# rusty-fast-solvers/rusty-compression

Measured on AMD Instinct MI355X. Metric: GB/s + compressions/sec, 8192x8192 f64 rank-128 rSVD+ID, higher is better.
Workload: dtype f64

## Files before the change

### rusty_compression_amd/csrc/kernels_gemm.hip

```cpp
#include "rc_common.hpp"
#include "rc_gemm.hpp"

#include <cstdlib>
#include <type_traits>

namespace rc {


constexpr int pitch16(int n) { return n + ((16 - n % 32) + 32) % 32; }
constexpr int pitch4(int n) { return n + ((4 - n % 8) + 8) % 8; }

template <typename T, int LAY, int R, int BK, int NT, int VEC, int MODE = 0>
struct TileStager {
    static constexpr int P = LAY == 0 ? (MODE == 0 ? BK + 2 : BK + 8) : (MODE == 0 ? pitch16(R) : pitch4(R));
    static constexpr int ELEMS = LAY == 0 ? R * P : BK * P;
    static constexpr int NVEC = R * BK / VEC;
    static constexpr int PER_T = (NVEC + NT - 1) / NT;
    typedef typename Acc<T>::vec2 vec2;

    const T *ptr[PER_T];
    T val[PER_T][VEC];

    static __device__ inline void coords(int idx, int &r, int &k) {
        if (LAY == 0) { k = (idx % (BK / VEC)) * VEC; r = idx / (BK / VEC); }
// ... 339 lines not shown
    }
}

template <typename T>
__global__ __launch_bounds__(256) void k_splitk_reduce_t(GemmArgs<T> g) {
    __shared__ T tile[32][33];
    const int tx = threadIdx.x & 31, ty = threadIdx.x >> 5;
    const int64_t n0 = (int64_t)blockIdx.x * 32, m0 = (int64_t)blockIdx.y * 32;
#pragma unroll
    for (int r = 0; r < 4; ++r) {
        const int64_t gm = m0 + ty + 8 * r, gn = n0 + tx;
        T s = 0;
        if (gm < g.M && gn < g.N) s = slab_sum(g.partial + gm * g.N + gn, g.M * g.N, g.splits);
        tile[ty + 8 * r][tx] = s;
    }
    __syncthreads();
#pragma unroll
    for (int r = 0; r < 4; ++r) {
        const int64_t gm = m0 + tx, gn = n0 + ty + 8 * r;
        if (gm < g.M && gn < g.N) {
            const T s = tile[tx][ty + 8 * r];
            T *cp = g.c + gm * g.scm + gn * g.scn;
            *cp = g.beta == (T)0 ? g.alpha * s : g.alpha * s + g.beta * (*cp);
        }
    }
}

static int wide_target(const rc_context *c, int many, int lone) {
    static const int target_slots = env_int("RC_GEMM_SLOTS_TARGET", 128);
    const int n = c->lanes_in_flight();
    return n >= 8 ? many : n >= 2 ? target_slots : lone;
}

template <typename T, int BK, class Pipe>
static void launch_split(rc_context *c, GemmArgs<T> g, int target, int min_ksteps, void (*kern)(GemmArgs<T>), int nt, size_t lds,
                         bool (&attr_set)[64], const char *name, Pipe &&pipe) {
    const int64_t tiles = (int64_t)g.tiles_m * g.tiles_n;
    int splits = 1;
    const int64_t ksteps = cdiv(g.K, BK);
    const int min_ks = min_ksteps > 0 ? min_ksteps : (tiles >= 32 ? 16 : 4);
    while (tiles * splits < target && splits < 128 && ksteps / (splits * 2) >= min_ks) splits *= 2;
    g.kchunk = cdiv(cdiv(g.K, splits), BK) * BK;
    splits = (int)cdiv(g.K, g.kchunk);
    if (splits < 1) splits = 1;
    g.splits = splits;
    ArenaMark mark(c);
    if (splits > 1) g.partial = c->alloc<T>((size_t)splits * g.M * g.N);
    if (lds > 48 * 1024 && !attr_set[c->device & 63]) {
        RC_HIP(hipFuncSetAttribute(reinterpret_cast<const void *>(kern), hipFuncAttributeMaxDynamicSharedMemorySize, (int)lds));
        attr_set[c->device & 63] = true;
    }
    c->last_gemm_kernel = name;
    if (!pipe(g)) {
        ProfScope ps(c, "kernel:k_gemm_mfma<%s> M=%lld N=%lld K=%lld", sizeof(T) == 8 ? "f64" : "f32", (long long)g.M, (long long)g.N, (long long)g.K);
        hipLaunchKernelGGL(kern, dim3((unsigned)tiles, (unsigned)splits), dim3(nt), lds, c->stream, g);
    }
    if (splits > 1) {
        ProfScope ps(c, "kernel:k_splitk_reduce M=%lld N=%lld splits=%d", (long long)g.M, (long long)g.N, splits);
        if (g.scm < g.scn && g.N >= 32) {
            hipLaunchKernelGGL(k_splitk_reduce_t<T>, dim3((unsigned)cdiv(g.N, 32), (unsigned)cdiv(g.M, 32)), dim3(256), 0, c->stream, g);
        } else {
            int grid = (int)std::min<int64_t>(cdiv(g.M * g.N, 256), 4096);
            hipLaunchKernelGGL(k_splitk_reduce<T>, dim3(grid), dim3(256), 0, c->stream, g);
        }
    }
}

template <typename T, int ALAY, int BLAY, int BM, int BN, int BK, int WM, int WN, int VEC, int NBUF = 2>
static void launch_cfg(rc_context *c, GemmArgs<T> g, int target_wgs = 0, int min_ksteps = 0) {
    constexpr int NT = WM * WN * 64;
    typedef TileStager<T, ALAY, BM, BK, NT, VEC> StA;
    typedef TileStager<T, BLAY == 1 ? 0 : 1, BN, BK, NT, VEC> StB;
    constexpr size_t lds = NBUF * (size_t)(StA::ELEMS + StB::ELEMS) * sizeof(T);
    static_assert(lds <= 160 * 1024, "tile does not fit LDS");
    g.tiles_m = (int)cdiv(g.M, BM);
    g.tiles_n = (int)cdiv(g.N, BN);
    const int64_t tiles = (int64_t)g.tiles_m * g.tiles_n;
    static const int target_big = env_int("RC_GEMM_TARGET_WGS", 256), target_small = env_int("RC_GEMM_SMALL_TARGET", 32);
    const int target = target_wgs > 0 ? target_wgs : tiles >= 8 ? (tiles >= 32 ? wide_target(c, 1, target_big) : target_big) : target_small;
    static bool attr_set[64] = {};
    char nm[128];
    snprintf(nm, sizeof(nm), "k_gemm_mfma<%s,%d,%d,%d,%d,%d,%d,%d,%d,%d>", sizeof(T) == 8 ? "double" : "float", ALAY, BLAY, BM, BN, BK, WM, WN, VEC, NBUF);
    launch_split<T, BK>(c, g, target, min_ksteps, k_gemm_mfma<T, ALAY, BLAY, BM, BN, BK, WM, WN, VEC, NBUF>, NT, lds, attr_set, nm,
                        [](const GemmArgs<T> &) { return false; });
}

template <int ALAY, int BLAY, int BM, int BN, int BK, int WM, int WN, int VEC, int ORIENT, int GLDS = 0>
static void launch_f64q(rc_context *c, GemmArgs<double> g, int target_wgs = 0, int min_ksteps = 0) {
    typedef double T;
    constexpr int NT = WM * WN * 64;
    typedef TileStager<T, ALAY, BM, BK, NT, VEC> StA;
    typedef TileStager<T, BLAY == 1 ? 0 : 1, BN, BK, NT, VEC> StB;
    constexpr size_t lds = 2 * (size_t)(StA::ELEMS + StB::ELEMS) * sizeof(T);
    static_assert(lds <= 160 * 1024, "tile does not fit LDS");
    g.tiles_m = (int)cdiv(g.M, BM);
    g.tiles_n = (int)cdiv(g.N, BN);
    const int64_t tiles = (int64_t)g.tiles_m * g.tiles_n;
    static const int target_big = env_int("RC_GEMM_TARGET_WGS", 256), target_small = env_int("RC_GEMM_SMALL_TARGET", 32);
    static const int target_lanes = env_int("RC_GEMM_LANES_TARGET", 1);
    const int lone = target_wgs > 0 ? target_wgs : target_big;
    const int target = tiles >= 8 ? (tiles >= 32 ? wide_target(c, target_lanes, lone) : lone) : target_small;
    static bool attr_set[64] = {};
    char nm[128];
    snprintf(nm, sizeof(nm), "k_gemm_f64q<%d,%d,%d,%d,%d,%d,%d,%d,%d,%d>", ALAY, BLAY, BM, BN, BK, WM, WN, VEC, ORIENT, GLDS);
    launch_split<T, BK>(c, g, target, min_ksteps, k_gemm_f64q<ALAY, BLAY, BM, BN, BK, WM, WN, VEC, ORIENT, GLDS>, NT, lds, attr_set, nm,
                        [&](const GemmArgs<T> &gs) { return gemm_f64p_launch(c, gs, ALAY, BLAY, BM, BN, BK, WM, WN, ORIENT, VEC == 2); });
}

template <int ALAY, int BLAY, int VEC>
static void launch_shape_f64q(rc_context *c, const GemmArgs<double> &g) {
    if (g.M <= 144 && g.N <= 144 && g.M > 80 && g.N > 80) launch_f64q<ALAY, BLAY, 144, 144, 16, 3, 3, VEC, 0>(c, g);
    else if (g.N <= 80) launch_f64q<ALAY, BLAY, 256, 80, 16, 8, 1, VEC, 0>(c, g);
    else if (g.N <= 128) launch_f64q<ALAY, BLAY, 256, 128, 16, 8, 1, VEC, 0>(c, g);
    else if (g.N <= 144) launch_f64q<ALAY, BLAY, 256, 144, 16, 8, 1, VEC, 0>(c, g);
    else if (g.M <= 32 && g.K >= 512) {
        launch_f64q<ALAY, BLAY, 32, 256, 16, 1, 8, VEC, 1>(c, g, 512, 4);
    }
    else if (g.M <= 80) launch_f64q<ALAY, BLAY, 80, 256, 16, 1, 8, VEC, 1>(c, g);
    else if (g.M <= 136 && g.K <= 160 && g.N >= 2048) {
        if (g.M <= 128) launch_f64q<ALAY, BLAY, 128, 128, 16, 1, 8, VEC, 1>(c, g);
        else launch_f64q<ALAY, BLAY, 136, 128, 16, 2, 4, VEC, 0>(c, g);
    }
    else if (g.M <= 128) {
        if constexpr (BLAY == 0 && VEC == 2) {
            const bool direct = g.N % 256 == 0 && g.K % 16 == 0 && g.sbn == 1 && g.sbk % 2 == 0 && reinterpret_cast<uintptr_t>(g.b) % 16 == 0;
            if constexpr (ALAY == 1) {
                const bool direct_a = g.M == 128 && g.sam == 1 && g.sak % 2 == 0 && reinterpret_cast<uintptr_t>(g.a) % 16 == 0;
                if (direct && direct_a) { launch_f64q<ALAY, BLAY, 128, 256, 16, 1, 8, VEC, 1, 2>(c, g); return; }
            }
            if (direct) { launch_f64q<ALAY, BLAY, 128, 256, 16, 1, 8, VEC, 1, 1>(c, g); return; }
        }
        launch_f64q<ALAY, BLAY, 128, 256, 16, 1, 8, VEC, 1>(c, g);
    }
    else if (g.M <= 136) launch_f64q<ALAY, BLAY, 136, 256, 16, 2, 4, VEC, 0>(c, g);
    else if (g.M <= 144) launch_f64q<ALAY, BLAY, 144, 256, 16, 1, 8, VEC, 1>(c, g);
    else launch_f64q<ALAY, BLAY, 128, 128, 16, 2, 2, VEC, 0>(c, g);
}

template <typename T, int ALAY, int BLAY, int VEC>
static void launch_shape(rc_context *c, const GemmArgs<T> &g) {
    if constexpr (std::is_same_v<T, double>) {
        launch_shape_f64q<ALAY, BLAY, VEC>(c, g);
    } else {
        constexpr bool panel = ALAY == 0 && BLAY == 1 && VEC == 2;
        if (g.M <= 144 && g.N <= 144 && g.M > 80 && g.N > 80) launch_cfg<T, ALAY, BLAY, 144, 144, 16, 3, 3, VEC>(c, g);
        else if (g.N <= 80) launch_cfg<T, ALAY, BLAY, 128, 80, 16, 4, 1, VEC>(c, g);
        else if (g.N <= 144) launch_cfg<T, ALAY, BLAY, 256, 144, 16, 8, 1, VEC>(c, g);
        else if (panel && g.M <= 32 && g.K >= 512) {
            if constexpr (panel) launch_cfg<T, ALAY, BLAY, 32, 128, 16, 1, 4, VEC>(c, g, 512, 4);
        } else if (g.M <= 80) launch_cfg<T, ALAY, BLAY, 80, 128, 16, 1, 4, VEC>(c, g);
        else if (g.M <= 144) launch_cfg<T, ALAY, BLAY, 144, 256, 16, 1, 8, VEC>(c, g);
        else launch_cfg<T, ALAY, BLAY, 128, 128, 16, 2, 2, VEC>(c, g);
    }
}

template <typename T, int ALAY, int BLAY>
static void launch_vec(rc_context *c, const GemmArgs<T> &g) {
    auto ok = [](const T *p, int64_t s_contig, int64_t s_other) {
        return s_contig == 1 && (s_other % 2) == 0 && (reinterpret_cast<uintptr_t>(p) % (2 * sizeof(T))) == 0;
    };
    const bool va = ALAY == 0 ? ok(g.a, g.sak, g.sam) : ok(g.a, g.sam, g.sak);
    const bool vb = BLAY == 0 ? ok(g.b, g.sbn, g.sbk) : ok(g.b, g.sbk, g.sbn);
    if (va && vb) launch_shape<T, ALAY, BLAY, 2>(c, g);
    else launch_shape<T, ALAY, BLAY, 1>(c, g);
}

template <typename T>
__global__ __launch_bounds__(256) void k_scale_c(Mat<T> cm, T beta) {
    const int64_t total = cm.rows * cm.cols;
    for (int64_t e = blockIdx.x * (int64_t)256 + threadIdx.x; e < total; e += (int64_t)gridDim.x * 256) {
        const int64_t j = e / cm.rows, i = e - j * cm.rows;
        cm.at(i, j) = beta * cm.at(i, j);
    }
}

template <typename T>
void gemm(rc_context *c, T alpha, Mat<T> a, Mat<T> b, T beta, Mat<T> cm) {
    RC_REQUIRE(a.cols == b.rows && a.rows == cm.rows && b.cols == cm.cols, RC_INVALID_ARGUMENT,
               "gemm: shapes (%lld x %lld) * (%lld x %lld) -> (%lld x %lld)", (long long)a.rows, (long long)a.cols,
               (long long)b.rows, (long long)b.cols, (long long)cm.rows, (long long)cm.cols);
    if (cm.empty()) return;
    ArenaMark mark(c);
    if (a.cols == 0) {
        if (beta == (T)0) fill_zero(c, cm);
        else if (beta != (T)1) hipLaunchKernelGGL(k_scale_c<T>, dim3((unsigned)std::min<int64_t>(cdiv(cm.rows * cm.cols, 256), 8192)), dim3(256), 0, c->stream, cm, beta);
        return;
    }
    if (a.rs != 1 && a.cs != 1) {
        T *p = c->alloc<T>((size_t)a.rows * a.cols);
        Mat<T> pa = rowmajor(p, a.rows, a.cols, a.cols);
        copy_mat(c, a, pa);
        a = pa;
    }
    if (b.rs != 1 && b.cs != 1) {
        T *p = c->alloc<T>((size_t)b.rows * b.cols);
        Mat<T> pb = rowmajor(p, b.rows, b.cols, b.cols);
        copy_mat(c, b, pb);
        b = pb;
    }
    if (sizeof(T) == 8 && b.cols <= 144 && a.rows > 144) {
        const Mat<T> a2 = b.t(), b2 = a.t();
        a = a2;
        b = b2;
        cm = cm.t();
    }
    GemmArgs<T> g;
    g.a = a.p; g.b = b.p; g.c = cm.p;
    g.M = a.rows; g.N = b.cols; g.K = a.cols;
    g.sam = a.rs; g.sak = a.cs; g.sbk = b.rs; g.sbn = b.cs; g.scm = cm.rs; g.scn = cm.cs;
    g.alpha = alpha; g.beta = beta;
    g.kchunk = g.K; g.splits = 1; g.partial = nullptr; g.tiles_m = g.tiles_n = 0;
    const bool a_kc = (a.cs == 1);
    const bool b_nc = (b.cs == 1);
    if (a_kc) {
        if (b_nc) launch_vec<T, 0, 0>(c, g); else launch_vec<T, 0, 1>(c, g);
    } else {
        if (b_nc) launch_vec<T, 1, 0>(c, g); else launch_vec<T, 1, 1>(c, g);
    }
}

template void gemm<double>(rc_context *, double, Mat<double>, Mat<double>, double, Mat<double>);
template void gemm<float>(rc_context *, float, Mat<float>, Mat<float>, float, Mat<float>);

}
```

### rusty_compression_amd/csrc/kernels_gemm_pipe.hip

```cpp
#include "rc_gemm.hpp"

#include <type_traits>
#include <utility>

namespace rc {

typedef double pdouble2_t __attribute__((ext_vector_type(2)));
typedef unsigned int pint4_t __attribute__((ext_vector_type(4)));

constexpr int pp_pitch16(int n) { return n + ((16 - n % 32) + 32) % 32; }

template <int LAY, int R, int BK, int NT>
struct PipeStage {
    static constexpr int P = LAY == 0 ? BK + 2 : pp_pitch16(R);
    static constexpr int ELEMS = LAY == 0 ? R * P : BK * P;
    static constexpr int NVEC = R * BK / 2;
    static constexpr int PER_T = (NVEC + NT - 1) / NT;
    static_assert(PER_T * NT <= 2 * NVEC && R % 2 == 0 && BK % 2 == 0, "staging shape");

    uint32_t goff[PER_T];
    pint4_t val[PER_T];

    static __device__ inline void coords(int idx, int &r, int &k) {
        if (idx >= NVEC) idx -= NVEC;
// ... 389 lines not shown
                    g.partial[((int64_t)split * g.M + gm) * g.N + gn] = v;
                } else {
                    double *cp = g.c + gm * g.scm + gn * g.scn;
                    *cp = g.beta == 0.0 ? g.alpha * v : g.alpha * v + g.beta * (*cp);
                }
            }
        }
}

template <int BLAY, int ORIENT, int BM, int BN, int WM, int WN, bool MASKTAIL>
static bool launch_r(rc_context *c, const GemmArgs<double> &g) {
    constexpr int NT = WM * WN * 64;
    constexpr size_t lds = 3 * (size_t)(DirectRows<BM, 16, NT, MASKTAIL>::ELEMS + (BLAY == 0 ? DirectRows<BN, 16, NT>::ELEMS : DirectK<BN, 16, NT>::ELEMS)) * sizeof(double);
    static_assert(lds <= 160 * 1024, "ring does not fit LDS");
    if (g.sam != 1) return false;
    if (BLAY == 0 ? g.sbn != 1 : (g.sbk != 1 || g.N % BN != 0)) return false;
    const int64_t a_span = ((int64_t)256 * g.sam + g.kchunk * g.sak + 2) * 8;
    const int64_t b_span = ((int64_t)BN * g.sbn + g.kchunk * g.sbk + 2) * 8;
    if (a_span >= (1ll << 31) || b_span >= (1ll << 31) || g.sak < 0 || g.sbn < 0 || g.sbk < 0) return false;
    auto kern = k_gemm_f64r<BLAY, ORIENT, BM, BN, WM, WN, MASKTAIL>;
    static bool attr_set[64] = {};
    if (!attr_set[c->device & 63]) {
        RC_HIP(hipFuncSetAttribute(reinterpret_cast<const void *>(kern), hipFuncAttributeMaxDynamicSharedMemorySize, (int)lds));
        attr_set[c->device & 63] = true;
    }
    char nm[128];
    snprintf(nm, sizeof(nm), "k_gemm_f64r<%d,%d,%d,%d,%d,%d,%s,0>", BLAY, ORIENT, BM, BN, WM, WN, MASKTAIL ? "true" : "false");
    c->last_gemm_kernel = nm;
    ProfScope ps(c, "kernel:k_gemm_mfma<f64> M=%lld N=%lld K=%lld", (long long)g.M, (long long)g.N, (long long)g.K);
    hipLaunchKernelGGL(kern, dim3((unsigned)(g.tiles_m * g.tiles_n), (unsigned)g.splits), dim3(NT), lds, c->stream, g);
    return true;
}

template <int ALAY, int BLAY, int BM, int BN, int BK, int WM, int WN, int ORIENT>
static bool launch_p(rc_context *c, const GemmArgs<double> &g) {
    constexpr int NT = WM * WN * 64;
    typedef PipeStage<ALAY, BM, BK, NT> SA;
    typedef PipeStage<BLAY == 1 ? 0 : 1, BN, BK, NT> SB;
    constexpr size_t lds = 2 * (size_t)(SA::ELEMS + SB::ELEMS) * sizeof(double);
    static_assert(lds <= 160 * 1024, "tile does not fit LDS");
    const int64_t a_span = ((int64_t)BM * g.sam + g.kchunk * g.sak + 2) * 8;
    const int64_t b_span = ((int64_t)BN * g.sbn + g.kchunk * g.sbk + 2) * 8;
    if (a_span >= (1ll << 31) || b_span >= (1ll << 31) || g.sam < 0 || g.sak < 0 || g.sbn < 0 || g.sbk < 0) return false;
    auto kern = k_gemm_f64p<ALAY, BLAY, BM, BN, BK, WM, WN, ORIENT>;
    static bool attr_set[64] = {};
    if (lds > 48 * 1024 && !attr_set[c->device & 63]) {
        RC_HIP(hipFuncSetAttribute(reinterpret_cast<const void *>(kern), hipFuncAttributeMaxDynamicSharedMemorySize, (int)lds));
        attr_set[c->device & 63] = true;
    }
    char nm[128];
    snprintf(nm, sizeof(nm), "k_gemm_f64p<%d,%d,%d,%d,%d,%d,%d,%d>", ALAY, BLAY, BM, BN, BK, WM, WN, ORIENT);
    c->last_gemm_kernel = nm;
    ProfScope ps(c, "kernel:k_gemm_mfma<f64> M=%lld N=%lld K=%lld", (long long)g.M, (long long)g.N, (long long)g.K);
    hipLaunchKernelGGL(kern, dim3((unsigned)(g.tiles_m * g.tiles_n), (unsigned)g.splits), dim3(NT), lds, c->stream, g);
    return true;
}

bool gemm_f64p_launch(rc_context *c, const GemmArgs<double> &g, int alay, int blay, int bm, int bn, int bk, int wm, int wn, int orient, bool vec2) {
    if (!vec2 || bk != 16) return false;
    if (g.K % bk != 0 || g.kchunk % bk != 0 || g.K < bk) return false;
    if (alay == 1 && blay == 1 && bm == 136 && bn == 256 && wm == 2 && wn == 4 && orient == 0 && launch_r<1, 0, 136, 256, 2, 4, true>(c, g)) return true;
    if (alay == 1 && blay == 0 && bm == 128 && bn == 256 && wm == 1 && wn == 8 && orient == 1 && launch_r<0, 1, 128, 256, 1, 8, false>(c, g)) return true;
#define RC_PIPE_CASE(AL, BL, BM_, BN_, WM_, WN_, OR_)                                                              \
    if (alay == AL && blay == BL && bm == BM_ && bn == BN_ && wm == WM_ && wn == WN_ && orient == OR_)             \
        return launch_p<AL, BL, BM_, BN_, 16, WM_, WN_, OR_>(c, g);
    RC_PIPE_CASE(0, 1, 144, 144, 3, 3, 0)
    RC_PIPE_CASE(1, 0, 144, 144, 3, 3, 0)
    RC_PIPE_CASE(1, 1, 136, 256, 2, 4, 0)
    RC_PIPE_CASE(1, 0, 128, 256, 1, 8, 1)
#undef RC_PIPE_CASE
    return false;
}

}

namespace rc {
template __global__ void k_gemm_f64r<1, 0, 136, 256, 2, 4, true>(GemmArgs<double>);
template __global__ void k_gemm_f64r<0, 1, 128, 256, 1, 8, false>(GemmArgs<double>);
}
```

### rusty_compression_amd/csrc/kernels_tsqr.hip

```cpp
#include "rc_common.hpp"
#include "rc_device.hpp"

namespace rc {

template <typename T> __device__ inline T tiny_pivot();
template <> __device__ inline double tiny_pivot<double>() { return 1e-300; }
template <> __device__ inline float tiny_pivot<float>() { return 1e-30f; }

template <typename T>
__device__ inline T wave_sum64(T v) {
#pragma unroll
    for (int off = 32; off > 0; off >>= 1) v += __shfl_xor(v, off, 64);
    return v;
}
template <typename T>
__device__ inline T row_sum16(T v) {
#pragma unroll
    for (int off = 8; off > 0; off >>= 1) v += __shfl_xor(v, off, 64);
    return v;
}

template <typename T, int NT, bool FOLD>
__global__ __launch_bounds__(1024) void k_chol_inv(Mat<T> g, Mat<T> r_out, Mat<T> rinv_out, Mat<T> r1, int check_identity, T ident_tol, T skip_tol, int *flag) {
    extern __shared__ __attribute__((aligned(16))) char smem_raw[];
// ... 171 lines not shown
        attr_set[c->device & 63] = true;
    }
    hipLaunchKernelGGL(kern, dim3(1), dim3(1024), chol_lds<T>(g.rows), c->stream, g, r, rinv, r1, check_identity ? 1 : 0, ident_tol, skip_tol, flag);
}
template <typename T>
static void chol_inv(rc_context *c, Mat<T> g, Mat<T> r, Mat<T> rinv, Mat<T> r1, bool check_identity, T ident_tol, T skip_tol, int *flag) {
    const int64_t n = g.rows;
    RC_REQUIRE(n <= 224 && chol_lds<T>(n) <= 160 * 1024 - 1024, RC_INVALID_ARGUMENT, "chol_inv: n = %lld does not fit LDS", (long long)n);
    ProfScope ps(c, "op:chol_inv n=%lld", (long long)n);
#define RC_CI(NT_)                                                                                          \
    do {                                                                                                    \
        if (r1.empty()) chol_inv_launch<T, NT_, false>(c, g, r, rinv, r1, check_identity, ident_tol, skip_tol, flag); \
        else chol_inv_launch<T, NT_, true>(c, g, r, rinv, r1, check_identity, ident_tol, skip_tol, flag);    \
    } while (0)
    if (n <= 64) RC_CI(2);
    else if (n <= 160) RC_CI(5);
    else if constexpr (sizeof(T) == 4) RC_CI(7);
#undef RC_CI
}

template <typename T>
bool tsqr_supported(int64_t m, int64_t n) {
    const size_t small_lds = ((size_t)n * (n | 1) + 4 * (size_t)n) * sizeof(T) + (size_t)n * sizeof(int) + 256;
    return n >= 2 && m >= 4 * n && m >= 1024 && small_lds <= 160 * 1024 - 2048;
}

template <typename T>
void tsqr_cholqr2_factored(rc_context *c, Mat<T> y, Mat<T> q1, Mat<T> r2i, Mat<T> r, int *flag) {
    const int64_t m = y.rows, n = y.cols;
    ProfScope ps(c, "op:cholqr2 %lldx%lld", (long long)m, (long long)n);
    ArenaMark mark(c);
    Mat<T> g = rowmajor(c->alloc<T>((size_t)n * even_ld(n)), n, n, even_ld(n));
    Mat<T> r1 = rowmajor(c->alloc<T>((size_t)n * even_ld(n)), n, n, even_ld(n)), r1i = rowmajor(c->alloc<T>((size_t)n * even_ld(n)), n, n, even_ld(n));
    gemm<T>(c, 1, y.t(), y, 0, g);
    chol_inv<T>(c, g, r1, r1i, Mat<T>(), false, 0, 0, flag);
    gemm<T>(c, 1, y, r1i, 0, q1);
    gemm<T>(c, 1, q1.t(), q1, 0, g);
    static const int skip_ok = env_int("RC_CHOLQR_SKIP", 1);
    const T skip_tol = skip_ok ? (sizeof(T) == 8 ? (T)2.5e-14 : (T)1e-6) : (T)-1;
    chol_inv<T>(c, g, r, r2i, r1, true, (T)1e-2, skip_tol, flag);
}

template <typename T>
void tsqr_cholqr2(rc_context *c, Mat<T> y, Mat<T> q, Mat<T> r, int *flag) {
    const int64_t m = y.rows, n = y.cols;
    ArenaMark mark(c);
    Mat<T> q1 = rowmajor(c->alloc<T>((size_t)m * even_ld(n)), m, n, even_ld(n));
    Mat<T> r2i = rowmajor(c->alloc<T>((size_t)n * even_ld(n)), n, n, even_ld(n));
    tsqr_cholqr2_factored<T>(c, y, q1, r2i, r, flag);
    gemm<T>(c, 1, q1, r2i, 0, q);
}

template <typename T>
__device__ inline T safe_hypot(T a, T b) {
    a = fabs(a); b = fabs(b);
    const T w = max(a, b), z = min(a, b);
    if (z == (T)0) return w;
    const T q = z * fast_rcp(w);
    const T e = (T)1 + q * q;
    return w * (e * fast_rsqrt(e));
}
template <typename T>
__device__ inline T fast_sqrt_pos(T x) { return x > (T)0 ? x * fast_rsqrt(x) : (T)0; }

template <typename T, int NEJ, int LPP>
__device__ __forceinline__ void qrcp_small_apply(T *A, int ld, int n, int j, int grp, int ll, int ngrp, const int *jp, T *vn1, T *vn2, T tj, int pivot, bool safe) {
    const T *vcol = A + jp[j] * ld;
    T v[NEJ];
#pragma unroll
    for (int e = 0; e < NEJ; ++e) {
// ... 423 lines not shown
}

int tsqr_fold() {
    static const int fold = env_int("RC_TSQR_FOLD", 1);
    return fold;
}

template <typename T>
void qrcp_tall_fast(rc_context *c, Mat<T> y, int64_t k, bool pivot, Mat<T> q, Mat<T> r, int64_t *ind, int *flag) {
    const int64_t m = y.rows, n = y.cols;
    ProfScope ps(c, "op:qrcp_tall_fast %lldx%lld k=%lld pivot=%d", (long long)m, (long long)n, (long long)k, pivot ? 1 : 0);
    ArenaMark mark(c);
    const int fold = tsqr_fold();
    Mat<T> q1 = rowmajor(c->alloc<T>((size_t)m * even_ld(n)), m, n, even_ld(n));
    Mat<T> r1 = colmajor(c->alloc<T>((size_t)n * even_ld(n)), n, n, even_ld(n));
    Mat<T> r2i = rowmajor(c->alloc<T>((size_t)n * even_ld(n)), n, n, even_ld(n));
    if (fold) tsqr_cholqr2_factored<T>(c, y, q1, r2i, r1, flag);
    else tsqr_cholqr2<T>(c, y, q1, r1, flag);
    Mat<T> q2 = colmajor(c->alloc<T>((size_t)even_ld(n) * k), n, k, even_ld(n));
    Mat<T> rr = r.empty() ? rowmajor(c->alloc<T>((size_t)k * even_ld(n)), k, n, even_ld(n)) : r;
    Mat<T> qq = q.empty() ? rowmajor(c->alloc<T>((size_t)m * even_ld(k)), m, k, even_ld(k)) : q;
    if (!fold) {
        qrcp_small<T>(c, r1, k, pivot, ind, rr, q2, Mat<T>(), Mat<T>(), Mat<T>(), Mat<T>());
        gemm<T>(c, 1, q1, q2, 0, qq);
        householder_sign_fix<T>(c, qq, rr);
        return;
    }
    Mat<T> w = colmajor(c->alloc<T>((size_t)even_ld(n) * k), n, k, even_ld(n));
    Mat<T> top = colmajor(c->alloc<T>((size_t)even_ld(k) * k), k, k, even_ld(k));
    T *d = c->alloc<T>((size_t)k);
    qrcp_small<T>(c, r1, k, pivot, ind, rr, q2, r2i, q1.sub(0, k, 0, n), w, top);
    householder_signs<T>(c, top, d);
    scale_cols_rows<T>(c, w, rr, d);
    gemm<T>(c, 1, q1, w, 0, qq);
}

#define RC_INST(T)                                                                                               \
    template bool tsqr_supported<T>(int64_t, int64_t);                                                           \
    template void tsqr_cholqr2<T>(rc_context *, Mat<T>, Mat<T>, Mat<T>, int *);                                  \
    template void tsqr_cholqr2_factored<T>(rc_context *, Mat<T>, Mat<T>, Mat<T>, Mat<T>, int *);                 \
    template void qrcp_small<T>(rc_context *, Mat<T>, int64_t, bool, int64_t *, Mat<T>, Mat<T>, Mat<T>, Mat<T>, Mat<T>, Mat<T>); \
    template void small_tri_product<T>(rc_context *, Mat<T>, Mat<T>, Mat<T>);                                   \
    template void householder_sign_fix<T>(rc_context *, Mat<T>, Mat<T>);                                         \
    template void qrcp_tall_fast<T>(rc_context *, Mat<T>, int64_t, bool, Mat<T>, Mat<T>, int64_t *, int *);
RC_INST(double)
RC_INST(float)
#undef RC_INST

}
```

### rusty_compression_amd/csrc/rc_api.hip

```cpp
#include "rc_common.hpp"

#include <unistd.h>

#include <atomic>
#include <chrono>

#include <algorithm>
#include <cmath>

using namespace rc;

static constexpr size_t kAlign = 256;

void rc_context::retire_arena() {
    if (arena) {
        if (live_graphs > 0) retired.push_back(arena);
        else (void)hipFree(arena);
    }
    arena = nullptr;
    arena_size = 0;
}

void rc_context::swap_arena() {
    std::swap(arena, aux_arena.base);
// ... 303 lines not shown
void lapack_orgqr(rc_context *c, Mat<T> a, const T *tau, int64_t k, Mat<T> q) {
    const int64_t m = a.rows;
    RC_REQUIRE(k >= 0 && k <= std::min(m, a.cols) && q.rows == m && q.cols == k, RC_INVALID_ARGUMENT,
               "orgqr: need k <= min(m, n) reflectors in a and q of m x k");
    if (k == 0 || m == 0) return;
    RC_REQUIRE(tau != nullptr, RC_INVALID_ARGUMENT, "orgqr: null tau");
    ArenaMark mark(c);
    int64_t *ident = c->alloc<int64_t>((size_t)k);
    iota_i64(c, ident, k);
    Mat<T> w = a.sub(0, m, 0, k);
    if (!(w.rs == 1 && w.cs >= m)) {
        Mat<T> wc = tmp_colmajor<T>(c, m, k);
        copy_mat(c, w, wc);
        w = wc;
    }
    form_q_into(c, w, ident, tau, k, q);
}

template <typename T>
void svd_finish(rc_context *c, bool transposed, bool factored, Mat<T> qw, Mat<T> q1, Mat<T> r2i, Mat<T> uc, Mat<T> vc, const T *s, Mat<T> u, Mat<T> vt,
                bool u_in_place = false, Mat<T> small = Mat<T>()) {
    const int64_t r = uc.rows;
    complete_left_basis(c, uc, s);
    if (factored && small.empty()) {
        small = tmp_colmajor<T>(c, r, r);
        small_tri_product<T>(c, r2i, transposed ? vc : uc, small);
    }
    if (!transposed) {
        if (factored) gemm<T>(c, 1, q1, small, 0, u);
        else gemm<T>(c, 1, qw, uc, 0, u);
        copy_mat(c, vc.t(), vt);
    } else {
        if (!u_in_place) copy_mat(c, uc, u);
        if (factored) gemm<T>(c, 1, small.t(), q1.t(), 0, vt);
        else gemm<T>(c, 1, vc.t(), qw.t(), 0, vt);
    }
}

template <typename T>
void svd_core(rc_context *c, Mat<T> wt, bool transposed, Mat<T> u, T *s, Mat<T> vt) {
    const int64_t M = wt.rows, r = wt.cols;
    ArenaMark mark(c);
    Mat<T> core = tmp_colmajor<T>(c, r, r);
    Mat<T> qw, q1, r2i;
    bool done = false;
    const int fold = tsqr_fold();
    if (c->opt_tsqr && tsqr_supported<T>(M, r)) {
        if (fold) {
            q1 = rowmajor(c->alloc<T>((size_t)M * even_ld(r)), M, r, even_ld(r));
            r2i = rowmajor(c->alloc<T>((size_t)r * even_ld(r)), r, r, even_ld(r));
            done = run_certified(c, [&](int *flag) { tsqr_cholqr2_factored<T>(c, wt, q1, r2i, transposed ? core.t() : core, flag); });
        } else {
            qw = tmp_colmajor<T>(c, M, r);
            done = run_certified(c, [&](int *flag) { tsqr_cholqr2<T>(c, wt, qw, transposed ? core.t() : core, flag); });
        }
    }
    const bool factored = done && fold;
    if (!done) {
        qw = tmp_colmajor<T>(c, M, r);
        int64_t *jp = c->alloc<int64_t>((size_t)std::max<int64_t>(r, 1));
        T *tau = c->alloc<T>((size_t)std::max<int64_t>(r, 1));
        T *vn = c->alloc<T>((size_t)std::max<int64_t>(2 * r, 1));
        geqp3_inplace(c, wt, r, false, jp, tau, vn);
        extract_r(c, wt, jp, transposed ? core.t() : core);
        form_q(c, wt, jp, tau, r, qw);
    }
    Mat<T> vwork = tmp_colmajor<T>(c, r, r), uc = tmp_colmajor<T>(c, r, r), vc = tmp_colmajor<T>(c, r, r);
// ... 179 lines not shown
        if (!run_certified(c, [&](int *flag) { tsqr_cholqr2_factored<T>(c, b.t(), q1, r2i, core.t(), flag); })) return false;
    }
    Mat<T> ub = tmp_colmajor<T>(c, k, k), vc = tmp_colmajor<T>(c, k, k);
    Mat<T> qb = tmp_colmajor<T>(c, k, k);
    Mat<T> small = tmp_colmajor<T>(c, k, k);
    Mat<T> r = o.qr_r.data ? from_c<T>(o.qr_r) : tmp_rowmajor<T>(c, k, n);
    int64_t *ind = o.qr_ind ? o.qr_ind : c->alloc<int64_t>((size_t)n);
    T *tau = c->alloc<T>((size_t)k);
    Mat<T> wf = tmp_colmajor<T>(c, k, n);
    T *s = static_cast<T *>(o.s);
    bool qr_done, small_done = false;
    {
        ProfScope ps(c, "stage:qrcp of B | svd of the core");
        qr_done = run_certified(c, [&](int *flag) { geqp3_wide_coop_jacobi<T>(c, b, wf, k, ind, tau, flag, core, ub, s, vc); });
    }
    {
        ProfScope ps(c, "stage:qrcp of B + column_id");
        const bool want_cz = o.id_c.data || o.id_z.data;
        Mat<T> cm = from_c<T>(o.id_c), z = from_c<T>(o.id_z);
        const bool tails = qr_done && k < n && id_fused();
        if (tails) {
            if (want_cz)
                RC_REQUIRE(cm.rows == m && cm.cols == k && z.rows == k && z.cols == n, RC_INVALID_ARGUMENT, "column_id: c %lld x %lld, z %lld x %lld",
                           (long long)cm.rows, (long long)cm.cols, (long long)z.rows, (long long)z.cols);
            rsvd_id_tails(c, wf, ind, tau, qb, r, want_cz ? z : Mat<T>(), r2i, vc, small);
            small_done = true;
        } else if (qr_done) {
            extract_r(c, wf, ind, r);
            form_q(c, wf, ind, tau, k, qb);
        } else {
            qrcp_core(c, b, k, true, qb, r, ind);
        }
        Mat<T> q = o.qr_q.data ? from_c<T>(o.qr_q) : tmp_colmajor<T>(c, m, k);
        gemm<T>(c, 1, range, qb, 0, q);
        if (want_cz && tails) gemm<T>(c, 1, q, r.sub(0, k, 0, k), 0, cm);
        else if (want_cz) qr_column_id(c, q, r, ind, cm, z, true);
    }
    {
        ProfScope ps(c, "stage:svd of B + U=Q Ub");
        svd_finish(c, true, true, Mat<T>(), q1, r2i, ub, vc, s, ub, from_c<T>(o.vt), true, small_done ? small : Mat<T>());
        gemm<T>(c, 1, range, ub, 0, from_c<T>(o.u));
    }
    return true;
}

template <typename T>
void rsvd_id_consumers(rc_context *c, Mat<T> range, Mat<T> b, const rc_rsvd_id_out &o) {
    const int64_t m = range.rows, k = b.rows, n = b.cols;
    const bool want_id = o.id_c.data || o.id_z.data || o.qr_q.data || o.qr_r.data || o.qr_ind;
    const bool want_svd = o.u.data || o.s || o.vt.data;
    if (want_svd) RC_REQUIRE(o.u.data && o.s && o.vt.data, RC_INVALID_ARGUMENT, "rsvd_id: u, s, vt must be given together");
    if (want_id && want_svd && !c->opt_fork && fused_consumers_qualify<T>(c, k, n)) {
        RC_REQUIRE(!(o.id_c.data || o.id_z.data) || (o.id_c.data && o.id_z.data), RC_INVALID_ARGUMENT, "rsvd_id: id_c and id_z must be given together");
        if (rsvd_id_consumers_fused(c, range, b, o)) return;
    }
    Mat<T> wq;
    if (want_id && want_svd && c->opt_fork) {
        wq = tmp_colmajor<T>(c, k, n);
        copy_mat(c, b, wq);
    }
    Fork fork(c, want_svd && want_id);
    if (want_id) {
        ProfScope ps(c, "stage:qrcp of B + column_id");
        Mat<T> qb = tmp_colmajor<T>(c, k, k);
        Mat<T> r = o.qr_r.data ? from_c<T>(o.qr_r) : tmp_rowmajor<T>(c, k, n);
        int64_t *ind = o.qr_ind ? o.qr_ind : c->alloc<int64_t>((size_t)n);
        if (wq.p) qrcp_core(c, wq, k, true, qb, r, ind);
        else qrcp_core(c, b, k, true, qb, r, ind, want_svd);
        Mat<T> q = o.qr_q.data ? from_c<T>(o.qr_q) : tmp_colmajor<T>(c, m, k);
        gemm<T>(c, 1, range, qb, 0, q);
        if (o.id_c.data || o.id_z.data) {
            RC_REQUIRE(o.id_c.data && o.id_z.data, RC_INVALID_ARGUMENT, "rsvd_id: id_c and id_z must be given together");
            qr_column_id(c, q, r, ind, from_c<T>(o.id_c), from_c<T>(o.id_z), true);
        }
// ... 514 lines not shown
```

### rusty_compression_amd/csrc/rc_common.hpp

```cpp
#pragma once

#include <hip/hip_runtime.h>

#include <algorithm>
#include <cstdarg>
#include <cstdint>
#include <cstdio>
#include <cstring>
#include <exception>
#include <cstdlib>
#include <map>
#include <memory>
#include <string>
#include <vector>

#include "../../include/rusty_compression_amd.h"

namespace rc {

template <typename T>
struct Mat {
    T *p = nullptr;
    int64_t rows = 0, cols = 0, rs = 0, cs = 0;

// ... 189 lines not shown
    size_t bytes = n * sizeof(T);
    if (c->pinned_size < bytes) {
        if (c->pinned) RC_HIP(hipHostFree(c->pinned));
        c->pinned = nullptr;
        c->pinned_size = 0;
        size_t want = std::max<size_t>(bytes, 1 << 16);
        RC_HIP(hipHostMalloc(&c->pinned, want, hipHostMallocDefault));
        c->pinned_size = want;
    }
    RC_HIP(hipMemcpyAsync(c->pinned, dev, bytes, hipMemcpyDeviceToHost, c->stream));
    RC_HIP(hipStreamSynchronize(c->stream));
    std::memcpy(host, c->pinned, bytes);
}

template <typename T> void fill_gaussian(rc_context *c, Mat<T> out, uint64_t seed, uint64_t offset);
void philox_words(rc_context *c, uint32_t *out, int64_t n, uint64_t seed, uint64_t word_offset);
template <typename T> void copy_mat(rc_context *c, Mat<T> src, Mat<T> dst);
template <typename T> void fill_identity(rc_context *c, Mat<T> dst);
template <typename T> void fill_zero(rc_context *c, Mat<T> dst);
template <typename T> void scale_rows(rc_context *c, const T *s, Mat<T> src, Mat<T> dst);
template <typename T> void gather_cols(rc_context *c, Mat<T> src, const int64_t *idx, Mat<T> dst);
template <typename T> void column_id_from_qrcp(rc_context *c, Mat<T> a, Mat<T> w, int64_t k, const int64_t *jpvt, Mat<T> cm, Mat<T> z);
template <typename T> void id_z_from_r(rc_context *c, Mat<T> r, int64_t k, const int64_t *ind, Mat<T> z);
template <typename T> void id_z_from_r_checked(rc_context *c, Mat<T> r, int64_t k, const int64_t *ind, const int64_t *inv, Mat<T> z);
void invert_perm(rc_context *c, const int64_t *perm, int64_t n, int64_t *inv);
void fill_words(rc_context *c, void *p, size_t bytes, unsigned v);
void iota_i64(rc_context *c, int64_t *p, int64_t n);
template <typename T> void col_sumsq(rc_context *c, Mat<T> a, T *out);
template <typename T> void max_sqrt(rc_context *c, const T *v, int64_t n, T *out);
template <typename T> void fro_diff(rc_context *c, Mat<T> a, Mat<T> b, T *out2);
template <typename T> void adaptive_residual_update(rc_context *c, Mat<T> y, Mat<T> corr);

template <typename T> void gemm(rc_context *c, T alpha, Mat<T> a, Mat<T> b, T beta, Mat<T> cmat);
template <typename T> void complete_left_basis(rc_context *c, Mat<T> uc, const T *s);

template <typename T> void geqp3_inplace(rc_context *c, Mat<T> w, int64_t kmax, bool pivot, int64_t *jpvt, T *tau, T *vn);
template <typename T> bool geqp3_blocked_supported(int64_t m, int64_t n, int64_t kmax);
template <typename T> void geqp3_blocked(rc_context *c, Mat<T> w, int64_t kmax, int64_t *jpvt, T *tau, Mat<T> q_out, Mat<T> restore_from = Mat<T>());
template <typename T> struct BlockedQrcpJob;
template <typename T> struct QrbJobDelete { void operator()(BlockedQrcpJob<T> *job) const; };
template <typename T> using QrbJobPtr = std::unique_ptr<BlockedQrcpJob<T>, QrbJobDelete<T>>;
template <typename T> QrbJobPtr<T> qrb_begin(rc_context *c, Mat<T> w, int64_t kmax, int64_t *jpvt, T *tau);
template <typename T> void qrb_issue(BlockedQrcpJob<T> *job);
template <typename T> bool qrb_finish(BlockedQrcpJob<T> *job);
constexpr int kQrbOptMaxPanels = 16;
struct QrbOptimistic {
    enum Status { NotPossible, NoSlots, Issued } status = NotPossible;
    const struct QrbState *log = nullptr;
    int panels = 0;
    int nbp[kQrbOptMaxPanels] = {};
    bool broken = false;
    bool verified() const;
};
template <typename T> QrbOptimistic qrb_issue_optimistic(BlockedQrcpJob<T> *job);
template <typename T> bool column_id_blocked_route(rc_context *c, int64_t m, int64_t n, int64_t k);
template <typename T> void column_id_rank(rc_context *c, Mat<T> a, int64_t k, Mat<T> cm, Mat<T> z, int64_t *col_ind);
template <typename T> Mat<T> tmp_colmajor_pitch4(rc_context *c, int64_t rows, int64_t cols);
template <typename E>
struct PackedSlot {
    Mat<E> cm, z;
    int64_t *ind;
};
template <typename E>
inline PackedSlot<E> packed_slot(void *packed, int idx, int64_t m, int64_t n, int64_t k) {
    const size_t per = rc_batch_packed_bytes(m, n, k, (int32_t)sizeof(E));
    char *base = static_cast<char *>(packed) + (size_t)idx * per;
// ... 33 lines not shown
```

### rusty_compression_amd/csrc/rc_gemm.hpp

```cpp
#pragma once
#include "rc_common.hpp"

namespace rc {

typedef double double4_t __attribute__((ext_vector_type(4)));
typedef float float4_t __attribute__((ext_vector_type(4)));
typedef double double2_t __attribute__((ext_vector_type(2)));
typedef float float2_t __attribute__((ext_vector_type(2)));

template <typename T> struct Acc;
template <> struct Acc<double> {
    typedef double4_t type;
    typedef double2_t vec2;
    static __device__ inline type mfma(double a, double b, type c) { return __builtin_amdgcn_mfma_f64_16x16x4f64(a, b, c, 0, 0, 0); }
    static __device__ inline int row(int lane, int reg) { return (lane >> 4) + 4 * reg; }
};
template <> struct Acc<float> {
    typedef float4_t type;
    typedef float2_t vec2;
    static __device__ inline type mfma(float a, float b, type c) { return __builtin_amdgcn_mfma_f32_16x16x4f32(a, b, c, 0, 0, 0); }
    static __device__ inline int row(int lane, int reg) { return 4 * (lane >> 4) + reg; }
};

constexpr int BSI_ROWS = 32;
constexpr int BSI_COLS = 64;
constexpr int BSI_PK = BSI_ROWS + 2;
constexpr int BSI_PA = 80;
constexpr int BSI_A_ELEMS = BSI_ROWS * BSI_PA;
static_assert(BSI_A_ELEMS >= BSI_COLS * BSI_PK && BSI_PA >= BSI_COLS, "A chunk image");
__host__ __device__ constexpr int bsi_po(int l) {
    return (((l + 15) & ~15) & 16) ? ((l + 15) & ~15) : ((l + 15) & ~15) + 16;
}
__host__ __device__ constexpr int bsi_o_elems(int l) {
    return BSI_ROWS * bsi_po(l) > ((l + 15) & ~15) * BSI_PK ? BSI_ROWS * bsi_po(l) : ((l + 15) & ~15) * BSI_PK;
}

template <typename T>
struct GemmArgs {
    const T *a, *b;
    T *c;
    int64_t M, N, K;
    int64_t sam, sak;
    int64_t sbk, sbn;
    int64_t scm, scn;
    T alpha, beta;
    int64_t kchunk;
    int splits;
    T *partial;
    int tiles_m, tiles_n;
};

bool gemm_f64p_launch(rc_context *c, const GemmArgs<double> &g, int alay, int blay, int bm, int bn, int bk, int wm, int wn, int orient, bool vec2);

}
```

Baseline: 759.7.

## Spread chain GEMMs over smaller tiles while planning split-K on original tiles

Adds a gemm_chain entry used by the CholQR, QRCP and final U/V GEMMs. In the 144x144 and tall-skinny (M<=136, N>=2048) shapes it launches smaller tiles (48x48, 128x32, 136x64), so more workgroups cover the GPU, while split-K is still planned from the original larger tile count. The point is to fill more compute units on these latency-bound GEMMs in the rank-128 pipeline without adding split-K partials and reductions. The trade-off is less data reuse per tile and more redundant loads of the shared operand. It also adds new pipelined 48x48 kernel instantiations and an env switch to turn the path off.

Measured after the change: 769.5, median of 6. 1.3% higher.

```diff
diff --git a/rusty_compression_amd/csrc/kernels_gemm.hip b/rusty_compression_amd/csrc/kernels_gemm.hip
--- a/rusty_compression_amd/csrc/kernels_gemm.hip
+++ b/rusty_compression_amd/csrc/kernels_gemm.hip
@@ -395,10 +395,8 @@
     return n >= 8 ? many : n >= 2 ? target_slots : lone;
 }
 
-template <typename T, int BK, class Pipe>
-static void launch_split(rc_context *c, GemmArgs<T> g, int target, int min_ksteps, void (*kern)(GemmArgs<T>), int nt, size_t lds,
-                         bool (&attr_set)[64], const char *name, Pipe &&pipe) {
-    const int64_t tiles = (int64_t)g.tiles_m * g.tiles_n;
+template <typename T, int BK>
+static void plan_split(GemmArgs<T> &g, int64_t tiles, int target, int min_ksteps) {
     int splits = 1;
     const int64_t ksteps = cdiv(g.K, BK);
     const int min_ks = min_ksteps > 0 ? min_ksteps : (tiles >= 32 ? 16 : 4);
@@ -407,6 +405,12 @@
     splits = (int)cdiv(g.K, g.kchunk);
     if (splits < 1) splits = 1;
     g.splits = splits;
+}
+
+template <typename T, class Pipe>
+static void launch_split(rc_context *c, GemmArgs<T> g, void (*kern)(GemmArgs<T>), int nt, size_t lds, bool (&attr_set)[64], const char *name, Pipe &&pipe) {
+    const int64_t tiles = (int64_t)g.tiles_m * g.tiles_n;
+    const int splits = g.splits;
     ArenaMark mark(c);
     if (splits > 1) g.partial = c->alloc<T>((size_t)splits * g.M * g.N);
     if (lds > 48 * 1024 && !attr_set[c->device & 63]) {
@@ -444,11 +448,11 @@
     static bool attr_set[64] = {};
     char nm[128];
     snprintf(nm, sizeof(nm), "k_gemm_mfma<%s,%d,%d,%d,%d,%d,%d,%d,%d,%d>", sizeof(T) == 8 ? "double" : "float", ALAY, BLAY, BM, BN, BK, WM, WN, VEC, NBUF);
-    launch_split<T, BK>(c, g, target, min_ksteps, k_gemm_mfma<T, ALAY, BLAY, BM, BN, BK, WM, WN, VEC, NBUF>, NT, lds, attr_set, nm,
-                        [](const GemmArgs<T> &) { return false; });
-}
-
-template <int ALAY, int BLAY, int BM, int BN, int BK, int WM, int WN, int VEC, int ORIENT, int GLDS = 0>
+    plan_split<T, BK>(g, tiles, target, min_ksteps);
+    launch_split<T>(c, g, k_gemm_mfma<T, ALAY, BLAY, BM, BN, BK, WM, WN, VEC, NBUF>, NT, lds, attr_set, nm, [](const GemmArgs<T> &) { return false; });
+}
+
+template <int ALAY, int BLAY, int BM, int BN, int BK, int WM, int WN, int VEC, int ORIENT, int GLDS = 0, int PBM = BM, int PBN = BN>
 static void launch_f64q(rc_context *c, GemmArgs<double> g, int target_wgs = 0, int min_ksteps = 0) {
     typedef double T;
     constexpr int NT = WM * WN * 64;
@@ -456,9 +460,10 @@
     typedef TileStager<T, BLAY == 1 ? 0 : 1, BN, BK, NT, VEC> StB;
     constexpr size_t lds = 2 * (size_t)(StA::ELEMS + StB::ELEMS) * sizeof(T);
     static_assert(lds <= 160 * 1024, "tile does not fit LDS");
+    static_assert(PBM % BM == 0 && PBN % BN == 0, "the launched tiles cut the planned one");
     g.tiles_m = (int)cdiv(g.M, BM);
     g.tiles_n = (int)cdiv(g.N, BN);
-    const int64_t tiles = (int64_t)g.tiles_m * g.tiles_n;
+    const int64_t tiles = cdiv(g.M, PBM) * cdiv(g.N, PBN);
     static const int target_big = env_int("RC_GEMM_TARGET_WGS", 256), target_small = env_int("RC_GEMM_SMALL_TARGET", 32);
     static const int target_lanes = env_int("RC_GEMM_LANES_TARGET", 1);
     const int lone = target_wgs > 0 ? target_wgs : target_big;
@@ -466,8 +471,9 @@
     static bool attr_set[64] = {};
     char nm[128];
     snprintf(nm, sizeof(nm), "k_gemm_f64q<%d,%d,%d,%d,%d,%d,%d,%d,%d,%d>", ALAY, BLAY, BM, BN, BK, WM, WN, VEC, ORIENT, GLDS);
-    launch_split<T, BK>(c, g, target, min_ksteps, k_gemm_f64q<ALAY, BLAY, BM, BN, BK, WM, WN, VEC, ORIENT, GLDS>, NT, lds, attr_set, nm,
-                        [&](const GemmArgs<T> &gs) { return gemm_f64p_launch(c, gs, ALAY, BLAY, BM, BN, BK, WM, WN, ORIENT, VEC == 2); });
+    plan_split<T, BK>(g, tiles, target, min_ksteps);
+    launch_split<T>(c, g, k_gemm_f64q<ALAY, BLAY, BM, BN, BK, WM, WN, VEC, ORIENT, GLDS>, NT, lds, attr_set, nm,
+                    [&](const GemmArgs<T> &gs) { return gemm_f64p_launch(c, gs, ALAY, BLAY, BM, BN, BK, WM, WN, ORIENT, VEC == 2); });
 }
 
 template <int ALAY, int BLAY, int VEC>
@@ -500,9 +506,29 @@
     else launch_f64q<ALAY, BLAY, 128, 128, 16, 2, 2, VEC, 0>(c, g);
 }
 
+template <int ALAY, int BLAY, int VEC>
+static bool launch_spread_f64q(rc_context *c, const GemmArgs<double> &g) {
+    if (g.M <= 144 && g.N <= 144 && g.M > 80 && g.N > 80) {
+        if constexpr (VEC == 2 && ALAY != BLAY) {
+            if (!gemm_f64p_accepts(g, 144, 144, 16)) return false;
+            launch_f64q<ALAY, BLAY, 48, 48, 16, 4, 1, VEC, 0, 0, 144, 144>(c, g);
+            return true;
+        }
+        return false;
+    }
+    if (g.N <= 144 || g.M <= 80) return false;
+    if (g.M <= 136 && g.K <= 160 && g.N >= 2048) {
+        if (g.M <= 128) launch_f64q<ALAY, BLAY, 128, 32, 16, 4, 2, VEC, 1, 0, 128, 128>(c, g);
+        else launch_f64q<ALAY, BLAY, 136, 64, 16, 2, 4, VEC, 0, 0, 136, 128>(c, g);
+        return true;
+    }
+    return false;
+}
+
 template <typename T, int ALAY, int BLAY, int VEC>
-static void launch_shape(rc_context *c, const GemmArgs<T> &g) {
+static void launch_shape(rc_context *c, const GemmArgs<T> &g, bool spread) {
     if constexpr (std::is_same_v<T, double>) {
+        if (spread && launch_spread_f64q<ALAY, BLAY, VEC>(c, g)) return;
         launch_shape_f64q<ALAY, BLAY, VEC>(c, g);
     } else {
         constexpr bool panel = ALAY == 0 && BLAY == 1 && VEC == 2;
@@ -518,14 +544,14 @@
 }
 
 template <typename T, int ALAY, int BLAY>
-static void launch_vec(rc_context *c, const GemmArgs<T> &g) {
+static void launch_vec(rc_context *c, const GemmArgs<T> &g, bool spread) {
     auto ok = [](const T *p, int64_t s_contig, int64_t s_other) {
         return s_contig == 1 && (s_other % 2) == 0 && (reinterpret_cast<uintptr_t>(p) % (2 * sizeof(T))) == 0;
     };
     const bool va = ALAY == 0 ? ok(g.a, g.sak, g.sam) : ok(g.a, g.sam, g.sak);
     const bool vb = BLAY == 0 ? ok(g.b, g.sbn, g.sbk) : ok(g.b, g.sbk, g.sbn);
-    if (va && vb) launch_shape<T, ALAY, BLAY, 2>(c, g);
-    else launch_shape<T, ALAY, BLAY, 1>(c, g);
+    if (va && vb) launch_shape<T, ALAY, BLAY, 2>(c, g, spread);
+    else launch_shape<T, ALAY, BLAY, 1>(c, g, spread);
 }
 
 template <typename T>
@@ -538,7 +564,7 @@
 }
 
 template <typename T>
-void gemm(rc_context *c, T alpha, Mat<T> a, Mat<T> b, T beta, Mat<T> cm) {
+static void gemm_run(rc_context *c, T alpha, Mat<T> a, Mat<T> b, T beta, Mat<T> cm, bool spread) {
     RC_REQUIRE(a.cols == b.rows && a.rows == cm.rows && b.cols == cm.cols, RC_INVALID_ARGUMENT,
                "gemm: shapes (%lld x %lld) * (%lld x %lld) -> (%lld x %lld)", (long long)a.rows, (long long)a.cols,
                (long long)b.rows, (long long)b.cols, (long long)cm.rows, (long long)cm.cols);
@@ -576,13 +602,30 @@
     const bool a_kc = (a.cs == 1);
     const bool b_nc = (b.cs == 1);
     if (a_kc) {
-        if (b_nc) launch_vec<T, 0, 0>(c, g); else launch_vec<T, 0, 1>(c, g);
+        if (b_nc) launch_vec<T, 0, 0>(c, g, spread); else launch_vec<T, 0, 1>(c, g, spread);
     } else {
-        if (b_nc) launch_vec<T, 1, 0>(c, g); else launch_vec<T, 1, 1>(c, g);
-    }
+        if (b_nc) launch_vec<T, 1, 0>(c, g, spread); else launch_vec<T, 1, 1>(c, g, spread);
+    }
+}
+
+template <typename T>
+void gemm(rc_context *c, T alpha, Mat<T> a, Mat<T> b, T beta, Mat<T> cm) {
+    gemm_run<T>(c, alpha, a, b, beta, cm, false);
+}
+
+template <typename T>
+void gemm_chain(rc_context *c, T alpha, Mat<T> a, Mat<T> b, T beta, Mat<T> cm) {
+    bool spread = false;
+    if constexpr (std::is_same_v<T, double>) {
+        static const int on = env_int("RC_GEMM_SPREAD", 1);
+        spread = on != 0 && c->lanes_in_flight() < 8;
+    }
+    gemm_run<T>(c, alpha, a, b, beta, cm, spread);
 }
 
 template void gemm<double>(rc_context *, double, Mat<double>, Mat<double>, double, Mat<double>);
 template void gemm<float>(rc_context *, float, Mat<float>, Mat<float>, float, Mat<float>);
-
-}
+template void gemm_chain<double>(rc_context *, double, Mat<double>, Mat<double>, double, Mat<double>);
+template void gemm_chain<float>(rc_context *, float, Mat<float>, Mat<float>, float, Mat<float>);
+
+}
diff --git a/rusty_compression_amd/csrc/kernels_gemm_pipe.hip b/rusty_compression_amd/csrc/kernels_gemm_pipe.hip
--- a/rusty_compression_amd/csrc/kernels_gemm_pipe.hip
+++ b/rusty_compression_amd/csrc/kernels_gemm_pipe.hip
@@ -445,6 +445,16 @@
     return true;
 }
 
+static bool pipe_spans_ok(const GemmArgs<double> &g, int bm, int bn, int64_t kchunk) {
+    const int64_t a_span = ((int64_t)bm * g.sam + kchunk * g.sak + 2) * 8;
+    const int64_t b_span = ((int64_t)bn * g.sbn + kchunk * g.sbk + 2) * 8;
+    return a_span < (1ll << 31) && b_span < (1ll << 31) && g.sam >= 0 && g.sak >= 0 && g.sbn >= 0 && g.sbk >= 0;
+}
+
+bool gemm_f64p_accepts(const GemmArgs<double> &g, int bm, int bn, int bk) {
+    return bk == 16 && g.K % bk == 0 && g.K >= bk && pipe_spans_ok(g, bm, bn, g.K);
+}
+
 template <int ALAY, int BLAY, int BM, int BN, int BK, int WM, int WN, int ORIENT>
 static bool launch_p(rc_context *c, const GemmArgs<double> &g) {
     constexpr int NT = WM * WN * 64;
@@ -452,9 +462,7 @@
     typedef PipeStage<BLAY == 1 ? 0 : 1, BN, BK, NT> SB;
     constexpr size_t lds = 2 * (size_t)(SA::ELEMS + SB::ELEMS) * sizeof(double);
     static_assert(lds <= 160 * 1024, "tile does not fit LDS");
-    const int64_t a_span = ((int64_t)BM * g.sam + g.kchunk * g.sak + 2) * 8;
-    const int64_t b_span = ((int64_t)BN * g.sbn + g.kchunk * g.sbk + 2) * 8;
-    if (a_span >= (1ll << 31) || b_span >= (1ll << 31) || g.sam < 0 || g.sak < 0 || g.sbn < 0 || g.sbk < 0) return false;
+    if (!pipe_spans_ok(g, BM, BN, g.kchunk)) return false;
     auto kern = k_gemm_f64p<ALAY, BLAY, BM, BN, BK, WM, WN, ORIENT>;
     static bool attr_set[64] = {};
     if (lds > 48 * 1024 && !attr_set[c->device & 63]) {
@@ -479,6 +487,8 @@
         return launch_p<AL, BL, BM_, BN_, 16, WM_, WN_, OR_>(c, g);
     RC_PIPE_CASE(0, 1, 144, 144, 3, 3, 0)
     RC_PIPE_CASE(1, 0, 144, 144, 3, 3, 0)
+    RC_PIPE_CASE(0, 1, 48, 48, 4, 1, 0)
+    RC_PIPE_CASE(1, 0, 48, 48, 4, 1, 0)
     RC_PIPE_CASE(1, 1, 136, 256, 2, 4, 0)
     RC_PIPE_CASE(1, 0, 128, 256, 1, 8, 1)
 #undef RC_PIPE_CASE
diff --git a/rusty_compression_amd/csrc/kernels_tsqr.hip b/rusty_compression_amd/csrc/kernels_tsqr.hip
--- a/rusty_compression_amd/csrc/kernels_tsqr.hip
+++ b/rusty_compression_amd/csrc/kernels_tsqr.hip
@@ -227,10 +227,10 @@
     ArenaMark mark(c);
     Mat<T> g = rowmajor(c->alloc<T>((size_t)n * even_ld(n)), n, n, even_ld(n));
     Mat<T> r1 = rowmajor(c->alloc<T>((size_t)n * even_ld(n)), n, n, even_ld(n)), r1i = rowmajor(c->alloc<T>((size_t)n * even_ld(n)), n, n, even_ld(n));
-    gemm<T>(c, 1, y.t(), y, 0, g);
+    gemm_chain<T>(c, 1, y.t(), y, 0, g);
     chol_inv<T>(c, g, r1, r1i, Mat<T>(), false, 0, 0, flag);
-    gemm<T>(c, 1, y, r1i, 0, q1);
-    gemm<T>(c, 1, q1.t(), q1, 0, g);
+    gemm_chain<T>(c, 1, y, r1i, 0, q1);
+    gemm_chain<T>(c, 1, q1.t(), q1, 0, g);
     static const int skip_ok = env_int("RC_CHOLQR_SKIP", 1);
     const T skip_tol = skip_ok ? (sizeof(T) == 8 ? (T)2.5e-14 : (T)1e-6) : (T)-1;
     chol_inv<T>(c, g, r, r2i, r1, true, (T)1e-2, skip_tol, flag);
@@ -720,7 +720,7 @@
     qrcp_small<T>(c, r1, k, pivot, ind, rr, q2, r2i, q1.sub(0, k, 0, n), w, top);
     householder_signs<T>(c, top, d);
     scale_cols_rows<T>(c, w, rr, d);
-    gemm<T>(c, 1, q1, w, 0, qq);
+    gemm_chain<T>(c, 1, q1, w, 0, qq);
 }
 
 #define RC_INST(T)                                                                                               \
diff --git a/rusty_compression_amd/csrc/rc_api.hip b/rusty_compression_amd/csrc/rc_api.hip
--- a/rusty_compression_amd/csrc/rc_api.hip
+++ b/rusty_compression_amd/csrc/rc_api.hip
@@ -359,7 +359,7 @@
         copy_mat(c, vc.t(), vt);
     } else {
         if (!u_in_place) copy_mat(c, uc, u);
-        if (factored) gemm<T>(c, 1, small.t(), q1.t(), 0, vt);
+        if (factored) gemm_chain<T>(c, 1, small.t(), q1.t(), 0, vt);
         else gemm<T>(c, 1, vc.t(), qw.t(), 0, vt);
     }
 }
@@ -605,14 +605,14 @@
             qrcp_core(c, b, k, true, qb, r, ind);
         }
         Mat<T> q = o.qr_q.data ? from_c<T>(o.qr_q) : tmp_colmajor<T>(c, m, k);
-        gemm<T>(c, 1, range, qb, 0, q);
-        if (want_cz && tails) gemm<T>(c, 1, q, r.sub(0, k, 0, k), 0, cm);
+        gemm_chain<T>(c, 1, range, qb, 0, q);
+        if (want_cz && tails) gemm_chain<T>(c, 1, q, r.sub(0, k, 0, k), 0, cm);
         else if (want_cz) qr_column_id(c, q, r, ind, cm, z, true);
     }
     {
         ProfScope ps(c, "stage:svd of B + U=Q Ub");
         svd_finish(c, true, true, Mat<T>(), q1, r2i, ub, vc, s, ub, from_c<T>(o.vt), true, small_done ? small : Mat<T>());
-        gemm<T>(c, 1, range, ub, 0, from_c<T>(o.u));
+        gemm_chain<T>(c, 1, range, ub, 0, from_c<T>(o.u));
     }
     return true;
 }
diff --git a/rusty_compression_amd/csrc/rc_common.hpp b/rusty_compression_amd/csrc/rc_common.hpp
--- a/rusty_compression_amd/csrc/rc_common.hpp
+++ b/rusty_compression_amd/csrc/rc_common.hpp
@@ -245,6 +245,7 @@
 template <typename T> void adaptive_residual_update(rc_context *c, Mat<T> y, Mat<T> corr);
 
 template <typename T> void gemm(rc_context *c, T alpha, Mat<T> a, Mat<T> b, T beta, Mat<T> cmat);
+template <typename T> void gemm_chain(rc_context *c, T alpha, Mat<T> a, Mat<T> b, T beta, Mat<T> cmat);
 template <typename T> void complete_left_basis(rc_context *c, Mat<T> uc, const T *s);
 
 template <typename T> void geqp3_inplace(rc_context *c, Mat<T> w, int64_t kmax, bool pivot, int64_t *jpvt, T *tau, T *vn);
diff --git a/rusty_compression_amd/csrc/rc_gemm.hpp b/rusty_compression_amd/csrc/rc_gemm.hpp
--- a/rusty_compression_amd/csrc/rc_gemm.hpp
+++ b/rusty_compression_amd/csrc/rc_gemm.hpp
@@ -51,5 +51,6 @@
 };
 
 bool gemm_f64p_launch(rc_context *c, const GemmArgs<double> &g, int alay, int blay, int bm, int bn, int bk, int wm, int wn, int orient, bool vec2);
+bool gemm_f64p_accepts(const GemmArgs<double> &g, int bm, int bn, int bk);
 
 }
```
